# UM-Applied-Algorithms-Lab/AWRY

Hardware: AMD Instinct MI355X
Metric: k-mer count queries/sec (parallel_count, random 31-mers, index resident in HBM) (higher is better)
Workload: dtype u64

## Files before the change

### awry_amd/_lib.py

```python
import ctypes as C
import importlib.util
import os
import re

_HERE = os.path.dirname(os.path.abspath(__file__))
_SO = os.path.join(_HERE, "lib", "libawry_hip.so")
_HEADER = os.path.join(os.path.dirname(_HERE), "include", "awry_hip.h")
_lib = None


def lib_path():
    return _SO


class Pos(C.Structure):
    _fields_ = [("seq_idx", C.c_uint64), ("local_pos", C.c_uint64)]


class Range(C.Structure):
    _fields_ = [("start_ptr", C.c_uint64), ("end_ptr", C.c_uint64)]


class Anchor(C.Structure):
    _fields_ = [("q_begin", C.c_uint32), ("q_len", C.c_uint32), ("start_row", C.c_uint64), ("count", C.c_uint64)]
# ... 69 lines not shown
            "there is no CPU fallback for the search path." % _SO)
    _preload_hip_runtime()
    L = C.CDLL(_SO)
    vp, u64, u8, i32, cp = C.c_void_p, C.c_uint64, C.c_uint8, C.c_int, C.c_char_p
    u64p, u8p = C.POINTER(C.c_uint64), C.POINTER(C.c_uint8)
    vpp = C.POINTER(vp)

    def sig(name, res, *args):
        f = getattr(L, name)
        f.restype, f.argtypes = res, list(args)

    sig("awry_last_error", cp)
    sig("awry_build", i32, C.POINTER(BuildArgs), vpp)
    sig("awry_build_from_text", i32, vp, u64, i32, u64, u8, u64p, C.POINTER(cp), u64, vpp)
    sig("awry_build_from_text_on", i32, vp, u64, i32, u64, u8, u64p, C.POINTER(cp), u64, i32, vpp)
    sig("awry_load", i32, cp, vpp)
    sig("awry_save", i32, vp, cp)
    sig("awry_free", None, vp)
    sig("awry_set_devices", i32, vp, C.POINTER(i32), i32)
    sig("awry_set_seed_kmer_len", i32, vp, i32)
    sig("awry_seed_kmer_len", i32, vp)
    sig("awry_debug_set_count_kernel", i32, i32)
    sig("awry_debug_force_wide_rows", i32, i32)
    sig("awry_debug_set_max_blocks", i32, i32)
    sig("awry_debug_max_blocks", i32)
    sig("awry_debug_dense_sa", vp, vp, i32)
    sig("awry_debug_accelerators", i32, vp, i32, C.POINTER(DebugAccel))
    sig("awry_debug_seed_rung", vp, vp, i32, i32)
    sig("awry_debug_set_ctx_extra_cap", i32, i32)
    sig("awry_count_schedule", cp, vp, i32)
    sig("awry_num_devices", i32, vp)
    sig("awry_replica_device", i32, vp, i32)
    sig("awry_count_batch", i32, vp, vp, u64p, u64, u64p)
    sig("awry_count_packed_kmers", i32, vp, u64p, u64, i32, u64p)
    sig("awry_locate_batch", i32, vp, vp, u64p, u64, C.POINTER(u64p), C.POINTER(C.POINTER(Pos)), C.POINTER(u64p))
    sig("awry_free_buffer", None, vp)
    sig("awry_count_mismatch_batch", i32, vp, vp, u64p, u64, i32, u64p)
    sig("awry_locate_mismatch_batch", i32, vp, vp, u64p, u64, i32, C.POINTER(u64p), C.POINTER(C.POINTER(Pos)), C.POINTER(u64p),
        C.POINTER(u8p))
    sig("awry_dev_count_mismatch", i32, vp, i32, vp, vp, u64, i32, vp, vp, vp)
    sig("awry_dev_count_mismatch_tally", i32, vp, i32, vp, vp, u64, i32, vp, vp, vp, vp)
    u32 = C.c_uint32
    sig("awry_pattern_class", u32, i32, u8)
    sig("awry_count_pattern_batch", i32, vp, vp, u64p, u64, i32, u64p)
    sig("awry_locate_pattern_batch", i32, vp, vp, u64p, u64, i32, C.POINTER(u64p), C.POINTER(C.POINTER(Pos)), C.POINTER(u64p),
        C.POINTER(u8p))
# ... 111 lines not shown
```

### awry_amd/csrc/awry_hip.hip

```cpp
#include "dev_common.h"
#include "replica.h"
#include "accelerators.h"
#include "launchers.h"
#include "host_count.h"
#include "host_locate.h"
#include "batch_host.h"
#include "mismatch_host.h"
#include "anchor_host.h"
#include "chain_host.h"
#include "edit_host.h"
#include "chain_align_host.h"
#include "map_host.h"
#include "split_host.h"
#include "pair_host.h"
#include "prewarm.h"

namespace {

template <class T>
T* malloc_array(size_t n) {
  const size_t bytes = std::max<size_t>(1, n) * sizeof(T);
  void* p = nullptr;
  if (bytes >= (8u << 20)) {
    if (posix_memalign(&p, 2u << 20, bytes) != 0) p = nullptr;
// ... 201 lines not shown
        });
      for (auto& t : pool) t.join();
      for (auto& e : errs) if (e) std::rethrow_exception(e);
    }
    idx->reps = std::move(reps);
    for (auto& r : idx->reps) prewarm_host_paths(*r);
  });
}

int awry_set_seed_kmer_len(awry_index_t* idx, int k) {
  return guarded([&] {
    require(idx != nullptr, "null index");
    require(k >= -1 && k <= 17, "seed k-mer length must be in -1..17 (amino: ..7)");
    idx->seed_k_request = k;
    for (size_t s = 0; s < idx->reps.size(); s++) {
      Replica& r = replica(idx, (int)s);
      build_seed(idx, r, k < 0 ? default_seed_k(idx->host) : k);
      sync_seed_mode(idx, r);
    }
  });
}

int awry_debug_set_count_kernel(int mode) { g_count_kernel.store(mode); return AWRY_OK; }
int awry_debug_force_wide_rows(int on) { g_force_wide.store(on ? 1 : 0); return AWRY_OK; }
int awry_debug_set_max_blocks(int blocks) {
  if (blocks < 0) { g_last_error = "awry_debug_set_max_blocks: negative bound"; return AWRY_ERR_ARG; }
  g_max_blocks.store(blocks);
  return AWRY_OK;
}
int awry_debug_max_blocks(void) { return g_max_blocks.load(); }

const char* awry_count_schedule(const awry_index_t* idx, int L) {
  if (!idx || idx->reps.empty()) return "";
  const CountFacts f = count_facts(*idx->reps[0]);
  const uint64_t n = 1u << 20;
  return plan_name(L > 32 ? plan_reads(f, n, L, true, false) : plan_kmers(f, n, L, true, false));
}

int awry_seed_kmer_len(const awry_index_t* idx) { return idx && !idx->reps.empty() ? idx->reps[0]->seed_k : 0; }
int awry_num_devices(const awry_index_t* idx) { return idx ? (int)idx->reps.size() : 0; }
int awry_replica_device(const awry_index_t* idx, int slot) {
  return idx && slot >= 0 && slot < (int)idx->reps.size() ? idx->reps[slot]->device : -1;
}

int awry_count_batch(awry_index_t* idx, const uint8_t* qbytes, const uint64_t* qoff, uint64_t n, uint64_t* counts_out) {
  return guarded([&] {
// ... 1047 lines not shown
```

### awry_amd/csrc/kernels_nt2_kmer.hip.h

```cpp
#pragma once

namespace awry {

__device__ __forceinline__ void tally_flush(unsigned long long* __restrict__ tally, uint32_t t_probe, uint32_t t_step, uint32_t t_blk) {
  atomicAdd(&tally[0], (unsigned long long)t_probe);
  atomicAdd(&tally[1], (unsigned long long)t_step);
  atomicAdd(&tally[2], (unsigned long long)t_blk);
}

template <bool USE_SEED, bool TALLY>
__global__ __launch_bounds__(256) void count_nt2_quad_kernel(DevIndex ix, const uint64_t* __restrict__ queries, uint64_t n, int L,
                                                             uint64_t* __restrict__ counts, unsigned long long* __restrict__ tally) {
  const int l = threadIdx.x & 3;
  const uint64_t nquads = ((uint64_t)gridDim.x * blockDim.x) >> 2;
  uint64_t q = ((uint64_t)blockIdx.x * blockDim.x + threadIdx.x) >> 2;
  const uint64_t* __restrict__ blocks = ix.blocks;
  const SeedEntry* __restrict__ seed = ix.seed;
  const int k = USE_SEED ? ix.seed_k : 1;
  const uint32_t cA = (uint32_t)ix.prefix_sums[1], cC = (uint32_t)ix.prefix_sums[2], cG = (uint32_t)ix.prefix_sums[3],
                 cN = (uint32_t)ix.prefix_sums[4], cT = (uint32_t)ix.prefix_sums[5], cEnd = (uint32_t)ix.prefix_sums[6];

  bool have = q < n;
  uint64_t w = have ? queries[q] : 0;
  bool fresh = true;
// ... 143 lines not shown
  if (TALLY && l == 0) {
    tally_flush(tally, t_probe, t_step, t_blk);
    atomicAdd(&tally[5], (unsigned long long)t_deep);
    if (VERIFY) {
      atomicAdd(&tally[3], (unsigned long long)t_vsa);
      atomicAdd(&tally[4], (unsigned long long)t_vtxt);
    }
  }
}

constexpr int VMULTI = 4;
constexpr int LCX_LANE_ROWS = 4;
constexpr int LCX_TAIL_MAX = 16;

struct Nt2Survivors {
  uint64_t* w;
  uint64_t* range;
  uint32_t* q;
  uint32_t* count;
  uint64_t cap;
  uint32_t* lf_count = nullptr;
};

template <bool TALLY, bool VERIFY>
__device__ __forceinline__ unsigned probe_block(const DevIndex& ix, const uint64_t* __restrict__ queries, uint64_t n, int L,
                                                uint64_t* __restrict__ counts, const Nt2Survivors& sv,
                                                unsigned long long* __restrict__ tally) {
  __shared__ unsigned int s_count;
  constexpr int VQ = 192;
  __shared__ uint64_t s_vw[VERIFY ? 4 : 1][VQ];
  __shared__ uint32_t s_vsp[VERIFY ? 4 : 1][VQ];
  __shared__ uint32_t s_vq[VERIFY ? 4 : 1][VQ];
  __shared__ uint8_t s_vn[VERIFY ? 4 : 1][VQ];
  if (threadIdx.x == 0) s_count = 0;
  if (blockIdx.x == 0 && threadIdx.x == 0 && sv.lf_count) *sv.lf_count = 0;
  __syncthreads();
  const int lane = threadIdx.x & 63, wv_id = threadIdx.x >> 6;
  const SeedEntry* __restrict__ seed = ix.seed;
  const int k = ix.seed_k, i0 = L - k, kshift = 2 * (L - k);
  const uint64_t kmask = (1ull << (2 * k)) - 1;
  const uint64_t stride = (uint64_t)gridDim.x * blockDim.x;
  const uint64_t lane_lt = (1ull << lane) - 1;
  const uint64_t region = (uint64_t)blockIdx.x * sv.cap;
  const bool pos = VERIFY && ix.seed_pos;
  const int cx = (int)ix.ctx_extra, clen = SEED_CTX_LEN + cx;
  const bool verify = VERIFY && (i0 >= 3 || (pos && i0 >= 1));
  const bool lcx = VERIFY && ix.lcx_key != nullptr && i0 >= 1;
  int vcount = 0;
  uint32_t t_vsa = 0, t_vtxt = 0, t_lcx = 0;
  auto drain = [&](int base, int cnt) {
    uint64_t w[2];
    uint32_t q[2], sp[2], nc[2], vp[2];
    bool on[2];
#pragma unroll
    for (int h = 0; h < 2; h++) {
      const int s = base + lane + 64 * h;
      on[h] = lane + 64 * h < cnt;
      w[h] = on[h] ? s_vw[VERIFY ? wv_id : 0][s] : 0;
      q[h] = on[h] ? s_vq[VERIFY ? wv_id : 0][s] : 0;
      sp[h] = on[h] ? s_vsp[VERIFY ? wv_id : 0][s] : 0;
      nc[h] = on[h] ? s_vn[VERIFY ? wv_id : 0][s] : 0;
      vp[h] = sp[h];
      if (on[h] && !(nc[h] & 0x80u) && !(pos && nc[h] == 1u)) { vp[h] = ix.dense_sa[sp[h]]; if (TALLY) t_vsa++; }
    }
#pragma unroll
    for (int h = 0; h < 2; h++) {
      if (!on[h]) continue;
      uint64_t value = 0;
      if (nc[h] & 0x80u) {
        const uint64_t want = (w[h] & ((1ull << (2 * i0)) - 1)) << (64 - 2 * i0);
        const uint32_t rows = nc[h] & 0x7Fu;
        const uint64_t* __restrict__ kp = ix.lcx_key + sp[h];
        const uint64_t k0 = kp[0], k1 = kp[1], k2 = rows > 2u ? kp[2] : ~want, k3 = rows > 3u ? kp[3] : ~want;
        const int sh = 64 - 2 * i0;
        value = (((k0 ^ want) >> sh) == 0) + (((k1 ^ want) >> sh) == 0) + (((k2 ^ want) >> sh) == 0) + (((k3 ^ want) >> sh) == 0);
        if (TALLY) t_lcx++;
        counts[q[h]] = value;
        continue;
      }
      for (uint32_t c = 0; c < nc[h]; c++) {
        const uint32_t p = c ? ix.dense_sa[sp[h] + c] : vp[h];
        if (TALLY && c) t_vsa++;
        if (p >= (uint32_t)i0) {
          if (TALLY) t_vtxt++;
          value += verify_part(ix.text4, (uint64_t)p - (uint64_t)i0, i0, 0, 0, w[h]) ? 0ull : 1ull;
        }
      }
      counts[q[h]] = value;
    }
  };
  constexpr int NQ = 4;
  for (uint64_t wbase = (uint64_t)blockIdx.x * blockDim.x + (threadIdx.x & ~63u); wbase < n; wbase += NQ * stride) {
    uint64_t qv[NQ], wv[NQ];
    SeedEntry ev[NQ];
#pragma unroll
    for (int h = 0; h < NQ; h++) {
      qv[h] = wbase + lane + (uint64_t)h * stride;
      wv[h] = qv[h] < n ? queries[qv[h]] : 0;
    }
#pragma unroll
    for (int h = 0; h < NQ; h++) {
      ev[h] = SeedEntry{1u, 0u};
      if (qv[h] < n) ev[h] = seed_probe(seed + ((wv[h] >> kshift) & kmask));
    }
#pragma unroll
    for (int h = 0; h < NQ; h++) {
      const bool valid = qv[h] < n;
      const uint64_t q = qv[h], w = wv[h];
      const SeedEntry e = ev[h];
      const uint32_t cnt = seed_cnt(e);
      bool survivor = false, queued = false, lcx_q = false;
      uint64_t value = 0;
      if (valid) {
        if (cnt == SEED_CNT_SAT) survivor = true;
        else if (cnt == 0u) value = 0;
        else if (i0 == 0) value = cnt;
        else if (cnt == 1u && pos && seed_has_ctx(e) && i0 <= clen) {
          value = (w & ((1ull << (2 * i0)) - 1)) == (seed_full_ctx(e, cx) >> (2 * (clen - i0))) ? 1ull : 0ull;
        } else if (cnt == 1u && pos && seed_has_ctx(e)) {
          queued = ((w >> (2 * (i0 - clen))) & ((1ull << (2 * clen)) - 1)) == seed_full_ctx(e, cx);
        } else if (cnt == 1u) {
          const uint32_t nc = (uint32_t)(w >> (2 * (i0 - 1))) & 3u;
          survivor = seed_sym(e) == (int)(nc == 3u ? 5u : nc + 1u);
          if (verify && survivor) { queued = true; survivor = false; }
        } else if (lcx && !(e.cnt & (SEED_LCX_NONE | SEED_LCX_TAIL)) && cnt <= (uint32_t)LCX_LANE_ROWS) {
          queued = true;
          lcx_q = true;
        } else if (lcx && !(e.cnt & SEED_LCX_NONE)) {
          survivor = true;
        } else if (verify && cnt <= (uint32_t)VMULTI && (int)(3u * cnt) <= i0 + 2) {
          queued = true;
        } else survivor = true;
        if (!queued) counts[q] = value;
      }
      if (VERIFY) {
        const uint64_t qm = __ballot(queued);
        if (qm) {
          if (queued) {
            const int s = vcount + (int)__popcll(qm & lane_lt);
            s_vw[wv_id][s] = w;
            s_vsp[wv_id][s] = cnt == 1u && pos ? seed_position(e, cx) : e.sp;
            s_vq[wv_id][s] = (uint32_t)q;
            s_vn[wv_id][s] = (uint8_t)(cnt | (lcx_q ? 0x80u : 0u));
          }
          vcount += (int)__popcll(qm);
          __builtin_amdgcn_wave_barrier();
          if (vcount >= 128) {
            vcount -= 128;
            drain(vcount, 128);
            __builtin_amdgcn_wave_barrier();
          }
        }
      }
      const uint64_t sm = __ballot(survivor);
      if (sm) {
        unsigned int slot0 = 0;
        if (lane == 0) slot0 = atomicAdd(&s_count, (unsigned int)__popcll(sm));
        slot0 = __shfl(slot0, 0, 64);
        if (survivor) {
          const uint64_t s = region + slot0 + (uint64_t)__popcll(sm & lane_lt);
          sv.w[s] = w;
          sv.range[s] = (uint64_t)e.sp | ((uint64_t)(cnt | (e.cnt & (SEED_LCX_NONE | SEED_LCX_TAIL))) << 32);
          sv.q[s] = (uint32_t)q;
        }
      }
    }
  }
  if (VERIFY && vcount > 0) drain(0, vcount);
  if (TALLY) {
    if (blockIdx.x == 0 && threadIdx.x == 0) atomicAdd(&tally[0], (unsigned long long)n);
    if (VERIFY && (t_vsa | t_vtxt | t_lcx)) {
      atomicAdd(&tally[3], (unsigned long long)t_vsa);
      atomicAdd(&tally[4], (unsigned long long)t_vtxt);
      atomicAdd(&tally[6], (unsigned long long)t_lcx);
    }
  }
  __syncthreads();
  return s_count;
}

template <bool TALLY, bool VERIFY>
__global__ __launch_bounds__(256) void count_nt2_probe_kernel(DevIndex ix, const uint64_t* __restrict__ queries, uint64_t n, int L,
                                                              uint64_t* __restrict__ counts, Nt2Survivors sv,
                                                              unsigned long long* __restrict__ tally) {
  const unsigned ns = probe_block<TALLY, VERIFY>(ix, queries, n, L, counts, sv, tally);
  if (threadIdx.x == 0) sv.count[blockIdx.x] = ns;
}

template <bool TALLY, bool VERIFY, bool TABLE = false>
__device__ __forceinline__ void resume_block_list(const DevIndex& ix, const Nt2Survivors& sv, uint64_t region, uint64_t ns, int L,
                                                  uint64_t* __restrict__ counts, unsigned long long* __restrict__ tally, bool allow_lcx,
                                                  uint64_t r_start, uint64_t r_stride) {
  const int l = threadIdx.x & 3;
  uint64_t r = r_start;
  const uint64_t* __restrict__ blocks = ix.blocks;
  const int k = ix.seed_k;
  const int verify_after = (int)ix.verify_after;
// ... 20 lines not shown
        if (fresh) {
          w = nx_w;
          const uint64_t rg = nx_rg;
          qidx = nx_q;
          if (r + r_stride < ns) { nx_w = sv.w[region + r + r_stride]; nx_rg = sv.range[region + r + r_stride]; nx_q = sv.q[region + r + r_stride]; }
          const uint32_t cf = (uint32_t)(rg >> 32), cnt = cf & SEED_CNT_SAT;
          steps_done = 0;
          fresh = false;
          if (qidx == 0xFFFFFFFFu) {
            sp = 1u; ep = 0u; i = 0;
          } else if (cnt == SEED_CNT_SAT) {
            const uint32_t c = (uint32_t)(w >> (2 * (L - 1))) & 3u;
            sp = c == 0 ? cA : (c == 1 ? cC : (c == 2 ? cG : cT));
            ep = (c == 0 ? cC : (c == 1 ? cG : (c == 2 ? cN : cEnd))) - 1;
            i = L - 1;
          } else {
            sp = (uint32_t)rg;
            ep = sp + cnt - 1u;
            i = L - k;
            if (lcx && cnt >= 2u && !(cf & SEED_LCX_NONE) && i > 0) {
              steps_done = 0;
              if (cf & SEED_LCX_TAIL) mode = 3;
              else { vp = ub_a = sp; vhits = ub_b = sp + cnt; vj = lcx_top_level(sp, cnt); mode = 4; }
              if (TABLE && ix.kmer_tab && cnt > (uint32_t)LCX_LANE_ROWS) { steps_done = mode; mode = 7; }
            }
          }
        }
        if (mode == 0) {
          const bool skip_step = VERIFY && i > 0 && sp <= ep && verify_now(ep - sp + 1u, i, steps_done, verify_after);
          if (i > 0 && sp <= ep && !skip_step) {
            i--;
            const uint32_t c = (uint32_t)(w >> (2 * i)) & 3u;
            const uint32_t cl = c == 0 ? cA : (c == 1 ? cC : (c == 2 ? cG : cT));
            if (TALLY) { t_step++; t_blk += ((sp - 1) >> 8) == (ep >> 8) ? 1u : 2u; }
            quad_step(blocks, cl, sp, ep, c, l);
            steps_done++;
          }
          if (sp > ep || i == 0) {
            finished = true;
            out_count = sp > ep ? 0ull : (uint64_t)(ep - sp) + 1ull;
          } else if (VERIFY) {
            const uint32_t cnt = ep - sp + 1u;
            if (verify_now(cnt, i, steps_done, verify_after)) { mode = 1; vj = 0; vhits = 0; }
          }
        }
      } else if (mode == 1) {
        vp = ix.dense_sa[sp + (uint32_t)vj];
// ... 68 lines not shown
    }
  }
  if (TALLY && l == 0) {
    atomicAdd(&tally[1], (unsigned long long)t_step);
    atomicAdd(&tally[2], (unsigned long long)t_blk);
    if (VERIFY) {
      atomicAdd(&tally[3], (unsigned long long)t_vsa);
      atomicAdd(&tally[4], (unsigned long long)t_vtxt);
      atomicAdd(&tally[6], (unsigned long long)t_lcx);
      atomicAdd(&tally[7], (unsigned long long)t_rp);
    }
  }
}

template <bool TALLY, bool VERIFY>
__global__ __launch_bounds__(256) void count_nt2_resume_kernel(DevIndex ix, Nt2Survivors sv, int L, uint64_t* __restrict__ counts,
                                                               unsigned long long* __restrict__ tally) {
  resume_block_list<TALLY, VERIFY>(ix, sv, (uint64_t)blockIdx.x * sv.cap, (uint64_t)sv.count[blockIdx.x], L, counts, tally, true, threadIdx.x >> 2, 64);
}

template <bool TALLY, bool VERIFY>
__global__ __launch_bounds__(256) void count_nt2_probe_resume_kernel(DevIndex ix, const uint64_t* __restrict__ queries, uint64_t n, int L, uint64_t* __restrict__ counts,
                                   Nt2Survivors sv, unsigned long long* __restrict__ tally) {
  const unsigned ns = probe_block<TALLY, VERIFY>(ix, queries, n, L, counts, sv, tally);
  resume_block_list<TALLY, VERIFY, true>(ix, sv, (uint64_t)blockIdx.x * sv.cap, (uint64_t)ns, L, counts, tally, true, threadIdx.x >> 2, 64);
}
constexpr int NT2_CHUNK = 256;

template <bool USE_SEED, bool TALLY>
__global__ __launch_bounds__(256) void count_nt2_chunk_kernel(DevIndex ix, const uint64_t* __restrict__ queries, uint64_t n, int L,
                                                              uint64_t* __restrict__ counts, unsigned long long* __restrict__ chunk_counter,
                                                              unsigned long long* __restrict__ tally) {
  __shared__ uint64_t lds_all[4 * NT2_CHUNK];
  const int lane = threadIdx.x & 63, l = lane & 3;
  volatile uint64_t* lds = lds_all + (threadIdx.x >> 6) * NT2_CHUNK;
  const uint64_t* __restrict__ blocks = ix.blocks;
  const SeedEntry* __restrict__ seed = ix.seed;
  const int k = USE_SEED ? ix.seed_k : 1;
  const uint32_t cA = (uint32_t)ix.prefix_sums[1], cC = (uint32_t)ix.prefix_sums[2], cG = (uint32_t)ix.prefix_sums[3],
                 cN = (uint32_t)ix.prefix_sums[4], cT = (uint32_t)ix.prefix_sums[5], cEnd = (uint32_t)ix.prefix_sums[6];
  const uint64_t nchunks = (n + NT2_CHUNK - 1) / NT2_CHUNK;
  const uint64_t quad_lt = (1ull << (lane & ~3)) - 1;
  uint32_t t_probe = 0, t_step = 0, t_blk = 0;

  for (;;) {
    unsigned long long c = 0;
    if (lane == 0) c = atomicAdd(chunk_counter, 1ull);
// ... 69 lines not shown
```

### awry_amd/csrc/kmer_table.hip.h

```cpp
#pragma once

namespace awry {

__device__ __forceinline__ void kt_add(uint64_t* __restrict__ table, uint32_t bits, uint64_t key, int L, uint64_t n, unsigned long long* __restrict__ stats) {
  const uint64_t mx = kt_mix(key, L);
  unsigned long long* line = reinterpret_cast<unsigned long long*>(table) + ((mx & ((1ull << bits) - 1)) << 4);
  const uint64_t tag = mx >> bits;
  for (int u = tag >= KT_TAG_NONE ? 16 : 0; u < 16;) {
    const unsigned long long e = __hip_atomic_load(line + u, __ATOMIC_RELAXED, __HIP_MEMORY_SCOPE_AGENT);
    const uint64_t cnt = e & KT_CNT_MASK;
    if (cnt == 0) {
      const uint64_t c = n < KT_ASK ? n : KT_ASK;
      if (atomicCAS(line + u, e, (tag << KT_TAG_SHIFT) | (e & KT_OVERFLOW) | c) == e) { atomicAdd(&stats[0], 1ull); return; }
      continue;
    }
    if ((e >> KT_TAG_SHIFT) == tag) {
      const uint64_t c = cnt + n < KT_ASK ? cnt + n : KT_ASK;
      if (atomicCAS(line + u, e, (e & ~KT_CNT_MASK) | c) == e) return;
      continue;
    }
    u++;
  }
  if (!(atomicOr(line, (unsigned long long)KT_OVERFLOW) & KT_OVERFLOW)) atomicAdd(&stats[1], 1ull);
}

template <bool INSERT>
__global__ __launch_bounds__(256) void kt_scan_kernel(DevIndex ix, int L, uint64_t* __restrict__ table, uint32_t bits, unsigned long long* __restrict__ stats) {
  const int k = ix.seed_k, i0 = L - k, sh = 64 - 2 * i0;
  const uint64_t stride = (uint64_t)gridDim.x * blockDim.x;
  unsigned long long mine = 0;
  for (uint64_t r = (uint64_t)blockIdx.x * blockDim.x + threadIdx.x; r < ix.bwt_len; r += stride) {
    const uint32_t p = ix.dense_sa[r];
    bool ok = false;
    const uint64_t kmer = lcx_text_letters(ix.text4, p, k, &ok);
    if (!ok) continue;
    const SeedEntry e = ix.seed[kmer];
    if (seed_has_ctx(e) || (e.cnt & SEED_LCX_NONE)) continue;
    const uint32_t cnt = e.cnt & SEED_CNT_SAT;
    if (cnt <= (uint32_t)LCX_LANE_ROWS || cnt == SEED_CNT_SAT) continue;
    const uint32_t sp = e.sp, j = (uint32_t)r - sp;
    if (r < sp || j >= cnt) continue;
    const uint32_t inc = (e.cnt & SEED_LCX_TAIL) ? (uint32_t)ix.lcx_key[sp + cnt - 1u] : 0u;
    const uint32_t nc = cnt - (inc < cnt ? inc : cnt);
    if (j < nc) {
// ... 31 lines not shown
```

### awry_amd/csrc/launchers.h

```cpp
#pragma once

namespace {

std::atomic<int> g_count_kernel{-1};
int count_kernel_override() {
  int m = g_count_kernel.load();
  if (m >= 0) return m;
  const char* e = getenv("AWRY_COUNT_KERNEL");
  if (e && !strcmp(e, "strided")) return 0;
  if (e && !strcmp(e, "chunk")) return 1;
  if (e && !strcmp(e, "quad4")) return 2;
  if (e && !strcmp(e, "twophase")) return 3;
  return -1;
}

CountFacts count_facts(const Replica& r) {
  static const bool rungs_off = getenv("AWRY_SEED_RUNGS") && !strcmp(getenv("AWRY_SEED_RUNGS"), "0");
  static const bool table_off = getenv("AWRY_KMER_TABLE") && !strcmp(getenv("AWRY_KMER_TABLE"), "0");
  CountFacts f;
  f.alphabet = r.dev.alphabet;
  f.wide = r.wide;
  f.bwt_len = r.dev.bwt_len;
  f.seed_k = r.seed_k;
  f.seed = r.seed.p != nullptr;
  f.seed64 = r.dev.seed64 != nullptr;
  f.text4 = r.dev.text4 != nullptr;
  f.dense_ratio = r.dev.dense_ratio;
  f.lcx_key = r.dev.lcx_key != nullptr;
  f.kt_mode = r.kt_mode;
  f.verify_kmers = r.verify_kmers;
  f.num_cus = r.num_cus;
  for (int i = 0; i < 4; i++) f.probe_resume_per_cu[i] = r.probe_resume_per_cu[i];
  for (int i = 0; i < 2; i++) f.lcx_reads_grid[i] = r.lcx_reads_grid[i];
  f.forced = count_kernel_override();
  f.rungs_off = rungs_off;
  f.table_off = table_off;
// ... 182 lines not shown
      });
      break;
    }
    default: require(false, "internal: not a schedule for reads");
  }
  HIP_CHECK(hipGetLastError());
}

void launch_count_nt2(Replica& r, const uint64_t* d_words, uint64_t n, int L, uint64_t* d_counts, bool use_seed, hipStream_t s,
                      unsigned long long* d_tally = nullptr) {
  require(r.dev.alphabet == NUCLEOTIDE, "packed 2-bit queries need a nucleotide index");
  require(L >= 1 && L <= 32, "packed k-mer length must be in 1..32");
  if (n == 0) return;
  const ScratchLock scratch_lock(r, s);
  CountFacts f = count_facts(r);
  CountPlan p = plan_kmers(f, n, L, use_seed, d_tally != nullptr);
  DevIndex dv = r.dev;
  std::shared_lock<std::shared_mutex> kt_lock;
  if (p.rung) {
    if (const SeedEntry* t = seed_rung(r, L)) { dv.seed = t; dv.seed_k = L; dv.seed_pos = 0; dv.ctx_extra = 0; }
    else { f.rung_failed = true; p = plan_kmers(f, n, L, use_seed, d_tally != nullptr); }
  }
  if (p.table) {
    if (const Replica::KmerTable* kt = kmer_table(r, L, true, kt_lock)) { dv.kmer_tab = kt->tab.p; dv.kmer_tab_bits = kt->bits; }
    else { f.table_failed = true; p = plan_kmers(f, n, L, use_seed, d_tally != nullptr); }
  }
  const dim3 g(plan_grid(r, p, n)), b(256);
  switch (p.schedule) {
    case CountSchedule::WIDE_SINGLE:
    case CountSchedule::WIDE_TWO_PHASE:
      launch_count_nt2_wide(r, p, d_words, n, L, d_counts, nullptr, s, nullptr, d_tally);
      return;
    case CountSchedule::LDS_CHUNKS: {
      unsigned long long* ctr = next_counter(r, s);
      with_flags(p.seeded, d_tally != nullptr, [&](auto S, auto T) {
        hipLaunchKernelGGL((count_nt2_chunk_kernel<S(), T()>), g, b, 0, s, r.dev, d_words, n, L, d_counts, ctr, d_tally);
      });
      break;
    }
    case CountSchedule::PROBE_RESUME:
    case CountSchedule::PROBE_THEN_RESUME: {
      Nt2Survivors sv, fb;
      two_phase_lists(r, s, n, p.blocks, 0u, &sv, &fb);
      with_flags(d_tally != nullptr, p.verify, [&](auto T, auto V) {
        if (p.schedule == CountSchedule::PROBE_THEN_RESUME) {
          hipLaunchKernelGGL((count_nt2_probe_kernel<T(), V()>), g, b, 0, s, dv, d_words, n, L, d_counts, sv, d_tally);
          hipLaunchKernelGGL((count_nt2_resume_kernel<T(), V()>), g, b, 0, s, dv, sv, L, d_counts, d_tally);
// ... 339 lines not shown
```

### awry_amd/csrc/layout.h

```cpp
#pragma once
#include <stdint.h>

#if defined(__HIP__)
#define AWRY_HD __host__ __device__ inline __attribute__((always_inline))
#else
#define AWRY_HD inline
#endif

namespace awry {

enum : int { NUCLEOTIDE = 0, AMINO = 1 };

constexpr int NT_BLOCK_WORDS = 16;
constexpr int AA_BLOCK_WORDS = 32;
constexpr int SYMBOLS_PER_BLOCK = 256;

AWRY_HD int block_words(int alphabet) { return alphabet == NUCLEOTIDE ? NT_BLOCK_WORDS : AA_BLOCK_WORDS; }
AWRY_HD int num_planes(int alphabet) { return alphabet == NUCLEOTIDE ? 3 : 5; }
AWRY_HD int cardinality(int alphabet) { return alphabet == NUCLEOTIDE ? 6 : 22; }

AWRY_HD int plane_word(int alphabet, int b, int l) {
  if (alphabet == NUCLEOTIDE) return b < 2 ? 2 * l + b : 8 + 2 * l;
  return b < 2 ? 2 * l + b : (b < 4 ? 8 + 2 * l + (b - 2) : 16 + 2 * l);
}
// ... 48 lines not shown
  const uint64_t* sa_words;
  const SeedEntry* seed;
  const SeedEntry64* seed64;
  const uint64_t* seq_starts;
  const uint32_t* seq_bucket;
  uint32_t seq_bucket_shift, seq_bucket_pad;
  uint64_t nblocks, bwt_len, sentinel_row, nseq;
  uint64_t prefix_sums[24];
  uint32_t sa_bits, sa_ratio;
  int32_t alphabet, seed_k;
  const uint32_t* dense_sa;
  const uint32_t* text4;
  uint32_t dense_ratio;
  uint32_t verify_after;
  const uint8_t* text8;
  uint32_t ctx_extra;
  uint32_t seed_pos;
  const uint32_t* sa_nblock;
  const uint64_t* lcx_key;
  const uint64_t* lcx_rowpos;
  const uint64_t* lcx_inner;
  uint32_t lcx_off[8];
  const uint64_t* kmer_tab;
  uint32_t kmer_tab_bits, kmer_tab_pad;
};
constexpr int LCX_CTX = 32;

constexpr int KT_CNT_BITS = 20, KT_TAG_SHIFT = 21, KT_TAG_BITS = 64 - KT_TAG_SHIFT;
constexpr uint64_t KT_CNT_MASK = (1ull << KT_CNT_BITS) - 1, KT_ASK = KT_CNT_MASK, KT_OVERFLOW = 1ull << KT_CNT_BITS;
constexpr uint64_t KT_TAG_NONE = (1ull << KT_TAG_BITS) - 1;
AWRY_HD uint64_t kt_mix(uint64_t w, int L) {
  const uint64_t m = L >= 32 ? ~0ull : (1ull << (2 * L)) - 1;
  w = (w * 0x9E3779B97F4A7C15ull) & m;
  w ^= w >> L;
  w = (w * 0xD6E8FEB86659FD93ull) & m;
  w ^= w >> L;
  return w;
}

constexpr uint64_t RS_MODE_SHIFT = 62;
constexpr uint64_t RS_PLAIN = 0;
constexpr uint64_t RS_MULTI = 1;
constexpr uint64_t RS_SINGLE = 2;
constexpr uint64_t RS_LCX = 3;

constexpr int LIST_MAX_LISTS = 4096;
constexpr int LCX_LF_CHUNK = 256;

}
```

### awry_amd/fm_index.py

```python
import ctypes as C
import os
from dataclasses import dataclass
from typing import Iterable, List, Optional, Sequence

import numpy as np

from . import _lib

NUCLEOTIDE, AMINO = 0, 1
BUILD_HOST, BUILD_AUTO = -1, -2


class SymbolAlphabet:
    Nucleotide = NUCLEOTIDE
    Amino = AMINO


class AwryError(RuntimeError):
    def __init__(self, code, msg):
        super().__init__("awry error %d: %s" % (code, msg))
        self.code = code


ERR_IO, ERR_FORMAT, ERR_INVALID_QUERY, ERR_HIP, ERR_OOM, ERR_ARG, ERR_NO_DEVICE = -1, -2, -3, -4, -5, -6, -7
# ... 939 lines not shown
    def dev_locate_tally(self, d_ranges, d_hit_off, n, total, d_gpos, d_pos, d_tally, stream=None, slot=0, range_stride=2):
        _check(self._L.awry_dev_locate_tally(self._h, slot, d_ranges, range_stride, d_hit_off, n, total, d_gpos, d_pos, d_tally, stream))

    def dev_phase_marker(self, phase_id, stream=None, slot=0):
        _check(self._L.awry_dev_phase_marker(self._h, slot, phase_id, stream))

    def dev_count_nt2_long(self, d_words, n, L, d_counts, d_range_start=None, use_seed=True, stream=None, slot=0):
        _check(self._L.awry_dev_count_nt2_long(self._h, slot, d_words, n, L, d_counts, d_range_start, 1 if use_seed else 0, stream))

    def set_locate_sa_ratio(self, ratio: int):
        _check(self._L.awry_set_locate_sa_ratio(self._h, ratio))

    def locate_sa_ratio(self) -> int:
        return self._L.awry_locate_sa_ratio(self._h)

    def set_lcx(self, on: bool):
        _check(self._L.awry_set_lcx(self._h, 1 if on else 0))

    def lcx_enabled(self) -> bool:
        return bool(self._L.awry_lcx_enabled(self._h))

    def set_kmer_table(self, mode: int):
        _check(self._L.awry_set_kmer_table(self._h, mode))

    def kmer_table_info(self, slot=0) -> dict:
        info = (C.c_uint64 * 6)()
        _check(self._L.awry_kmer_table_info(self._h, slot, info))
        return {"length": int(info[0]), "entries": int(info[1]), "lines": int(info[2]), "overflowed_lines": int(info[3]),
                "bytes": int(info[4]), "build_ms": int(info[5]) / 1000.0}

    def debug_kmer_table(self, slot=0):
        L, bits = C.c_int(0), C.c_uint32(0)
        for _ in range(4):
            _check(self._L.awry_debug_kmer_table(self._h, slot, None, 0, C.byref(L), C.byref(bits)))
            if L.value == 0:
                return None
            want = bits.value
            tab = np.empty(16 << want, np.uint64)
            _check(self._L.awry_debug_kmer_table(self._h, slot, tab.ctypes.data, len(tab), C.byref(L), C.byref(bits)))
            if L.value == 0:
                return None
            if bits.value <= want:
                return tab[:16 << bits.value], int(bits.value), int(L.value)
        raise AwryError(ERR_ARG, "the k-mer count table kept changing size while it was read")

    def debug_lcx(self, slot=0):
# ... 114 lines not shown
```

### include/awry_hip.h

```cpp
#ifndef AWRY_HIP_H
#define AWRY_HIP_H
#include <stddef.h>
#include <stdint.h>

#ifdef __cplusplus
extern "C" {
#endif

enum {
  AWRY_OK = 0,
  AWRY_ERR_IO = -1,
  AWRY_ERR_FORMAT = -2,
  AWRY_ERR_INVALID_QUERY = -3,
  AWRY_ERR_HIP = -4,
  AWRY_ERR_OOM = -5,
  AWRY_ERR_ARG = -6,
  AWRY_ERR_NO_DEVICE = -7
};

enum { AWRY_NUCLEOTIDE = 0, AWRY_AMINO = 1 };

typedef struct awry_index awry_index_t;

typedef struct { uint64_t seq_idx, local_pos; } awry_pos_t;
// ... 6 lines not shown
  uint64_t sa_ratio;
  uint8_t kmer_len;
  uint8_t alphabet;
  uint64_t max_query_len;
  uint8_t remove_tmp;
} awry_build_args_t;

int awry_build(const awry_build_args_t *args, awry_index_t **out);
int awry_build_from_text(const uint8_t *text, uint64_t bwt_len, int alphabet, uint64_t sa_ratio, uint8_t kmer_len,
                         const uint64_t *seq_starts, const char *const *headers, uint64_t nseq, awry_index_t **out);
enum { AWRY_BUILD_HOST = -1, AWRY_BUILD_AUTO = -2 };
int awry_build_from_text_on(const uint8_t *text, uint64_t bwt_len, int alphabet, uint64_t sa_ratio, uint8_t kmer_len,
                            const uint64_t *seq_starts, const char *const *headers, uint64_t nseq, int build_device,
                            awry_index_t **out);
int awry_load(const char *path, awry_index_t **out);
int awry_save(awry_index_t *idx, const char *path);
void awry_free(awry_index_t *idx);

int awry_set_devices(awry_index_t *idx, const int *device_ids, int n_devices);
int awry_set_seed_kmer_len(awry_index_t *idx, int k);
int awry_seed_kmer_len(const awry_index_t *idx);
int awry_debug_set_count_kernel(int mode);
int awry_debug_force_wide_rows(int on);
int awry_debug_set_max_blocks(int blocks);
int awry_debug_max_blocks(void);
const void *awry_debug_dense_sa(const awry_index_t *idx, int slot);
typedef struct {
  const void *seed;
  int32_t seed_k, seed_entry_bytes, seed_pos, ctx_extra;
  const void *dense_sa;
  uint64_t dense_ratio;
  const void *text4;
  uint64_t text4_words;
  const void *text8;
  const void *sa_nblock;
  uint64_t nblock_lo, nblock_hi;
  const void *lcx_inner;
  uint64_t lcx_inner_words;
  uint32_t lcx_off[8];
} awry_debug_accel_t;
int awry_debug_accelerators(const awry_index_t *idx, int slot, awry_debug_accel_t *out);
const void *awry_debug_seed_rung(awry_index_t *idx, int slot, int L);
int awry_debug_set_ctx_extra_cap(int cap);
const char *awry_count_schedule(const awry_index_t *idx, int L);
int awry_set_locate_sa_ratio(awry_index_t *idx, int ratio);
int awry_locate_sa_ratio(const awry_index_t *idx);
// ... 298 lines not shown
```

### rust/awry-hip-sys/src/lib.rs

```rust
#![allow(non_camel_case_types)]
use std::os::raw::{c_char, c_int, c_void};

pub const AWRY_OK: c_int = 0;
pub const AWRY_ERR_IO: c_int = -1;
pub const AWRY_ERR_FORMAT: c_int = -2;
pub const AWRY_ERR_INVALID_QUERY: c_int = -3;
pub const AWRY_ERR_HIP: c_int = -4;
pub const AWRY_ERR_OOM: c_int = -5;
pub const AWRY_ERR_ARG: c_int = -6;
pub const AWRY_ERR_NO_DEVICE: c_int = -7;
pub const AWRY_NUCLEOTIDE: c_int = 0;
pub const AWRY_AMINO: c_int = 1;
pub const AWRY_BUILD_HOST: c_int = -1;
pub const AWRY_BUILD_AUTO: c_int = -2;

#[repr(C)]
pub struct awry_index_t {
    _private: [u8; 0],
}

#[repr(C)]
#[derive(Clone, Copy, Debug, Default, PartialEq, Eq)]
pub struct awry_pos_t {
    pub seq_idx: u64,
// ... 146 lines not shown
pub struct awry_build_args_t {
    pub input_path: *const c_char,
    pub sa_tmp_path: *const c_char,
    pub sa_ratio: u64,
    pub kmer_len: u8,
    pub alphabet: u8,
    pub max_query_len: u64,
    pub remove_tmp: u8,
}

#[link(name = "awry_hip")]
extern "C" {
    pub fn awry_build(args: *const awry_build_args_t, out: *mut *mut awry_index_t) -> c_int;
    pub fn awry_build_from_text(text: *const u8, bwt_len: u64, alphabet: c_int, sa_ratio: u64, kmer_len: u8, seq_starts: *const u64, headers: *const *const c_char, nseq: u64, out: *mut *mut awry_index_t) -> c_int;
    pub fn awry_build_from_text_on(text: *const u8, bwt_len: u64, alphabet: c_int, sa_ratio: u64, kmer_len: u8, seq_starts: *const u64, headers: *const *const c_char, nseq: u64, build_device: c_int, out: *mut *mut awry_index_t) -> c_int;
    pub fn awry_load(path: *const c_char, out: *mut *mut awry_index_t) -> c_int;
    pub fn awry_save(idx: *mut awry_index_t, path: *const c_char) -> c_int;
    pub fn awry_free(idx: *mut awry_index_t);
    pub fn awry_set_devices(idx: *mut awry_index_t, device_ids: *const c_int, n_devices: c_int) -> c_int;
    pub fn awry_set_seed_kmer_len(idx: *mut awry_index_t, k: c_int) -> c_int;
    pub fn awry_seed_kmer_len(idx: *const awry_index_t) -> c_int;
    pub fn awry_debug_set_count_kernel(mode: c_int) -> c_int;
    pub fn awry_debug_force_wide_rows(on: c_int) -> c_int;
    pub fn awry_debug_set_max_blocks(blocks: c_int) -> c_int;
    pub fn awry_debug_max_blocks() -> c_int;
    pub fn awry_debug_dense_sa(idx: *const awry_index_t, slot: c_int) -> *const c_void;
    pub fn awry_debug_accelerators(idx: *const awry_index_t, slot: c_int, out: *mut awry_debug_accel_t) -> c_int;
    pub fn awry_debug_seed_rung(idx: *mut awry_index_t, slot: c_int, L: c_int) -> *const c_void;
    pub fn awry_debug_set_ctx_extra_cap(cap: c_int) -> c_int;
    pub fn awry_count_schedule(idx: *const awry_index_t, L: c_int) -> *const c_char;
    pub fn awry_set_locate_sa_ratio(idx: *mut awry_index_t, ratio: c_int) -> c_int;
    pub fn awry_locate_sa_ratio(idx: *const awry_index_t) -> c_int;
    pub fn awry_set_verify(idx: *mut awry_index_t, after_steps: c_int) -> c_int;
    pub fn awry_set_verify_kmers(idx: *mut awry_index_t, on: c_int) -> c_int;
    pub fn awry_verify_enabled(idx: *const awry_index_t) -> c_int;
    pub fn awry_set_lcx(idx: *mut awry_index_t, on: c_int) -> c_int;
    pub fn awry_lcx_enabled(idx: *const awry_index_t) -> c_int;
    pub fn awry_debug_lcx(idx: *const awry_index_t, slot: c_int, d_keys: *mut *const c_void, d_rowpos: *mut *const c_void) -> c_int;
    pub fn awry_set_kmer_table(idx: *mut awry_index_t, mode: c_int) -> c_int;
    pub fn awry_kmer_table_info(idx: *mut awry_index_t, slot: c_int, info: *mut u64) -> c_int;
    pub fn awry_debug_set_kmer_table_lines(lines: u64) -> c_int;
    pub fn awry_debug_kmer_table(idx: *mut awry_index_t, slot: c_int, host_out: *mut u64, capacity_words: u64, L_out: *mut c_int, bits_out: *mut u32) -> c_int;
    pub fn awry_num_devices(idx: *const awry_index_t) -> c_int;
    pub fn awry_count_batch(idx: *mut awry_index_t, qbytes: *const u8, qoff: *const u64, n: u64, counts_out: *mut u64) -> c_int;
    pub fn awry_count_packed_kmers(idx: *mut awry_index_t, words: *const u64, n: u64, L: c_int, counts_out: *mut u64) -> c_int;
    pub fn awry_locate_batch(idx: *mut awry_index_t, qbytes: *const u8, qoff: *const u64, n: u64, hit_off_out: *mut *mut u64, hits_out: *mut *mut awry_pos_t, global_pos_out: *mut *mut u64) -> c_int;
// ... 99 lines not shown
```

Before: 39.21 billion.

## Resolve k-mer hash-table lookups per lane in probe phase before survivor resume

Adds a per-lane k-mer count table lookup inside the probe block's drain step. Queries whose seed range exceeds the lane-row limit are queued for a direct table probe instead of being written out as survivors for the later resume phase. Only table misses, ask-markers and overflow cases fall back to the survivor list, tagged so resume does not look them up again. The table probe start slot is now spread by tag bits in both insert and lookup, to lower clustering within a 16-slot line. The change cuts survivor traffic and resume work, at the cost of extra register and shared-memory pressure and more divergent loops in the probe kernel.

```diff
diff --git a/awry_amd/_lib.py b/awry_amd/_lib.py
--- a/awry_amd/_lib.py
+++ b/awry_amd/_lib.py
@@ -115,6 +115,7 @@
     sig("awry_seed_kmer_len", i32, vp)
     sig("awry_debug_set_count_kernel", i32, i32)
     sig("awry_debug_force_wide_rows", i32, i32)
+    sig("awry_debug_set_kmer_lane_lookup", i32, i32)
     sig("awry_debug_set_max_blocks", i32, i32)
     sig("awry_debug_max_blocks", i32)
     sig("awry_debug_dense_sa", vp, vp, i32)
diff --git a/awry_amd/csrc/awry_hip.hip b/awry_amd/csrc/awry_hip.hip
--- a/awry_amd/csrc/awry_hip.hip
+++ b/awry_amd/csrc/awry_hip.hip
@@ -247,6 +247,7 @@
 }
 
 int awry_debug_set_count_kernel(int mode) { g_count_kernel.store(mode); return AWRY_OK; }
+int awry_debug_set_kmer_lane_lookup(int on) { g_kmer_lane.store(on < 0 ? -1 : (on ? 1 : 0)); return AWRY_OK; }
 int awry_debug_force_wide_rows(int on) { g_force_wide.store(on ? 1 : 0); return AWRY_OK; }
 int awry_debug_set_max_blocks(int blocks) {
   if (blocks < 0) { g_last_error = "awry_debug_set_max_blocks: negative bound"; return AWRY_ERR_ARG; }
diff --git a/awry_amd/csrc/kernels_nt2_kmer.hip.h b/awry_amd/csrc/kernels_nt2_kmer.hip.h
--- a/awry_amd/csrc/kernels_nt2_kmer.hip.h
+++ b/awry_amd/csrc/kernels_nt2_kmer.hip.h
@@ -189,7 +189,10 @@
   uint32_t* lf_count = nullptr;
 };
 
-template <bool TALLY, bool VERIFY>
+constexpr int KT_LANE_INFLIGHT = 2;
+constexpr uint32_t KT_QUEUED = 0x40u;
+constexpr uint32_t SV_TABLE_ASKED = 0x80000000u;
+template <bool TALLY, bool VERIFY, bool TABLE = false>
 __device__ __forceinline__ unsigned probe_block(const DevIndex& ix, const uint64_t* __restrict__ queries, uint64_t n, int L,
                                                 uint64_t* __restrict__ counts, const Nt2Survivors& sv,
                                                 unsigned long long* __restrict__ tally) {
@@ -213,8 +216,9 @@
   const int cx = (int)ix.ctx_extra, clen = SEED_CTX_LEN + cx;
   const bool verify = VERIFY && (i0 >= 3 || (pos && i0 >= 1));
   const bool lcx = VERIFY && ix.lcx_key != nullptr && i0 >= 1;
+  const bool kt_lane = TABLE && lcx && ix.kmer_tab != nullptr && ix.kmer_tab_lane != 0;
   int vcount = 0;
-  uint32_t t_vsa = 0, t_vtxt = 0, t_lcx = 0;
+  uint32_t t_vsa = 0, t_vtxt = 0, t_lcx = 0, t_kt = 0;
   auto drain = [&](int base, int cnt) {
     uint64_t w[2];
     uint32_t q[2], sp[2], nc[2], vp[2];
@@ -228,11 +232,11 @@
       sp[h] = on[h] ? s_vsp[VERIFY ? wv_id : 0][s] : 0;
       nc[h] = on[h] ? s_vn[VERIFY ? wv_id : 0][s] : 0;
       vp[h] = sp[h];
-      if (on[h] && !(nc[h] & 0x80u) && !(pos && nc[h] == 1u)) { vp[h] = ix.dense_sa[sp[h]]; if (TALLY) t_vsa++; }
+      if (on[h] && !(nc[h] & (0x80u | KT_QUEUED)) && !(pos && nc[h] == 1u)) { vp[h] = ix.dense_sa[sp[h]]; if (TALLY) t_vsa++; }
     }
 #pragma unroll
     for (int h = 0; h < 2; h++) {
-      if (!on[h]) continue;
+      if (!on[h] || (TABLE && (nc[h] & KT_QUEUED))) continue;
       uint64_t value = 0;
       if (nc[h] & 0x80u) {
         const uint64_t want = (w[h] & ((1ull << (2 * i0)) - 1)) << (64 - 2 * i0);
@@ -255,6 +259,69 @@
       }
       counts[q[h]] = value;
     }
+    if (TABLE && kt_lane && __any((nc[0] | nc[1]) & KT_QUEUED)) {
+      __asm__ volatile("" ::: "memory");
+      uint64_t kw[2];
+      uint32_t mark[2];
+      ulonglong2 x[2], y[2];
+      bool kt[2], back[2];
+      const uint64_t lmask = (1ull << ix.kmer_tab_bits) - 1;
+#pragma unroll
+      for (int g = 0; g < 2; g += KT_LANE_INFLIGHT) {
+#pragma unroll
+      for (int h = g; h < g + KT_LANE_INFLIGHT; h++) {
+        const int s = base + lane + 64 * h;
+        kt[h] = lane + 64 * h < cnt && (s_vn[VERIFY ? wv_id : 0][s] & KT_QUEUED);
+        if (!kt[h]) continue;
+        kw[h] = s_vw[VERIFY ? wv_id : 0][s];
+        const uint64_t mx = kt_mix(kw[h], L);
+        const uint64_t* line = ix.kmer_tab + ((mx & lmask) << 4);
+        const ulonglong2* sec = reinterpret_cast<const ulonglong2*>(line + kt_probe_slot(mx >> ix.kmer_tab_bits, 0));
+        mark[h] = *reinterpret_cast<const uint32_t*>(line);
+        x[h] = sec[0];
+        y[h] = sec[1];
+        if (TALLY) t_lcx++;
+      }
+#pragma unroll
+      for (int h = g; h < g + KT_LANE_INFLIGHT; h++) {
+        back[h] = false;
+        if (!kt[h]) continue;
+        const uint64_t mx = kt_mix(kw[h], L), tag = mx >> ix.kmer_tab_bits;
+        const uint64_t want = tag >= KT_TAG_NONE ? ~0ull : tag << KT_TAG_SHIFT;
+        uint32_t found = 0;
+        for (int j = 0;;) {
+          found = (((x[h].x ^ want) >> KT_TAG_SHIFT) == 0 ? (uint32_t)x[h].x & (uint32_t)KT_CNT_MASK : 0u) +
+                  (((x[h].y ^ want) >> KT_TAG_SHIFT) == 0 ? (uint32_t)x[h].y & (uint32_t)KT_CNT_MASK : 0u) +
+                  (((y[h].x ^ want) >> KT_TAG_SHIFT) == 0 ? (uint32_t)y[h].x & (uint32_t)KT_CNT_MASK : 0u) +
+                  (((y[h].y ^ want) >> KT_TAG_SHIFT) == 0 ? (uint32_t)y[h].y & (uint32_t)KT_CNT_MASK : 0u);
+          const bool empty = !((uint32_t)x[h].x & (uint32_t)KT_CNT_MASK) || !((uint32_t)x[h].y & (uint32_t)KT_CNT_MASK) ||
+                             !((uint32_t)y[h].x & (uint32_t)KT_CNT_MASK) || !((uint32_t)y[h].y & (uint32_t)KT_CNT_MASK);
+          j += 4;
+          if (found || empty || j == 16) break;
+          const ulonglong2* sec = reinterpret_cast<const ulonglong2*>(ix.kmer_tab + ((mx & lmask) << 4) + kt_probe_slot(tag, j));
+          x[h] = sec[0];
+          y[h] = sec[1];
+        }
+        back[h] = found == (uint32_t)KT_ASK || (found == 0u && (mark[h] & (uint32_t)KT_OVERFLOW));
+        if (!back[h]) { counts[s_vq[VERIFY ? wv_id : 0][base + lane + 64 * h]] = found; if (TALLY) t_kt++; }
+      }
+      }
+#pragma unroll
+      for (int h = 0; h < 2; h++) {
+        const uint64_t bm = __ballot(back[h]);
+        if (!bm) continue;
+        unsigned int slot0 = 0;
+        if (lane == 0) slot0 = atomicAdd(&s_count, (unsigned int)__popcll(bm));
+        slot0 = __shfl(slot0, 0, 64);
+        if (back[h]) {
+          const SeedEntry e = seed_probe(seed + ((kw[h] >> kshift) & kmask));
+          const uint64_t s = region + slot0 + (uint64_t)__popcll(bm & lane_lt);
+          sv.w[s] = kw[h];
+          sv.range[s] = (uint64_t)e.sp | ((uint64_t)((e.cnt & (SEED_CNT_SAT | SEED_LCX_NONE | SEED_LCX_TAIL)) | SV_TABLE_ASKED) << 32);
+          sv.q[s] = s_vq[VERIFY ? wv_id : 0][base + lane + 64 * h];
+        }
+      }
+    }
   };
   constexpr int NQ = 4;
   for (uint64_t wbase = (uint64_t)blockIdx.x * blockDim.x + (threadIdx.x & ~63u); wbase < n; wbase += NQ * stride) {
@@ -276,7 +343,7 @@
       const uint64_t q = qv[h], w = wv[h];
       const SeedEntry e = ev[h];
       const uint32_t cnt = seed_cnt(e);
-      bool survivor = false, queued = false, lcx_q = false;
+      bool survivor = false, queued = false, lcx_q = false, kt_q = false;
       uint64_t value = 0;
       if (valid) {
         if (cnt == SEED_CNT_SAT) survivor = true;
@@ -294,7 +361,8 @@
           queued = true;
           lcx_q = true;
         } else if (lcx && !(e.cnt & SEED_LCX_NONE)) {
-          survivor = true;
+          if (TABLE && kt_lane && cnt > (uint32_t)LCX_LANE_ROWS) queued = kt_q = true;
+          else survivor = true;
         } else if (verify && cnt <= (uint32_t)VMULTI && (int)(3u * cnt) <= i0 + 2) {
           queued = true;
         } else survivor = true;
@@ -308,7 +376,7 @@
             s_vw[wv_id][s] = w;
             s_vsp[wv_id][s] = cnt == 1u && pos ? seed_position(e, cx) : e.sp;
             s_vq[wv_id][s] = (uint32_t)q;
-            s_vn[wv_id][s] = (uint8_t)(cnt | (lcx_q ? 0x80u : 0u));
+            s_vn[wv_id][s] = TABLE && kt_q ? (uint8_t)KT_QUEUED : (uint8_t)(cnt | (lcx_q ? 0x80u : 0u));
           }
           vcount += (int)__popcll(qm);
           __builtin_amdgcn_wave_barrier();
@@ -340,6 +408,7 @@
       atomicAdd(&tally[3], (unsigned long long)t_vsa);
       atomicAdd(&tally[4], (unsigned long long)t_vtxt);
       atomicAdd(&tally[6], (unsigned long long)t_lcx);
+      if (TABLE && t_kt) atomicAdd(&tally[5], (unsigned long long)t_kt);
     }
   }
   __syncthreads();
@@ -406,7 +475,7 @@
               steps_done = 0;
               if (cf & SEED_LCX_TAIL) mode = 3;
               else { vp = ub_a = sp; vhits = ub_b = sp + cnt; vj = lcx_top_level(sp, cnt); mode = 4; }
-              if (TABLE && ix.kmer_tab && cnt > (uint32_t)LCX_LANE_ROWS) { steps_done = mode; mode = 7; }
+              if (TABLE && ix.kmer_tab && cnt > (uint32_t)LCX_LANE_ROWS && !(cf & SV_TABLE_ASKED)) { steps_done = mode; mode = 7; }
             }
           }
         }
@@ -521,7 +590,7 @@
 template <bool TALLY, bool VERIFY>
 __global__ __launch_bounds__(256) void count_nt2_probe_resume_kernel(DevIndex ix, const uint64_t* __restrict__ queries, uint64_t n, int L, uint64_t* __restrict__ counts,
                                    Nt2Survivors sv, unsigned long long* __restrict__ tally) {
-  const unsigned ns = probe_block<TALLY, VERIFY>(ix, queries, n, L, counts, sv, tally);
+  const unsigned ns = probe_block<TALLY, VERIFY, true>(ix, queries, n, L, counts, sv, tally);
   resume_block_list<TALLY, VERIFY, true>(ix, sv, (uint64_t)blockIdx.x * sv.cap, (uint64_t)ns, L, counts, tally, true, threadIdx.x >> 2, 64);
 }
 constexpr int NT2_CHUNK = 256;
diff --git a/awry_amd/csrc/kmer_table.hip.h b/awry_amd/csrc/kmer_table.hip.h
--- a/awry_amd/csrc/kmer_table.hip.h
+++ b/awry_amd/csrc/kmer_table.hip.h
@@ -6,7 +6,8 @@
   const uint64_t mx = kt_mix(key, L);
   unsigned long long* line = reinterpret_cast<unsigned long long*>(table) + ((mx & ((1ull << bits) - 1)) << 4);
   const uint64_t tag = mx >> bits;
-  for (int u = tag >= KT_TAG_NONE ? 16 : 0; u < 16;) {
+  for (int j = tag >= KT_TAG_NONE ? 16 : 0; j < 16;) {
+    const int u = kt_probe_slot(tag, j);
     const unsigned long long e = __hip_atomic_load(line + u, __ATOMIC_RELAXED, __HIP_MEMORY_SCOPE_AGENT);
     const uint64_t cnt = e & KT_CNT_MASK;
     if (cnt == 0) {
@@ -19,7 +20,7 @@
       if (atomicCAS(line + u, e, (e & ~KT_CNT_MASK) | c) == e) return;
       continue;
     }
-    u++;
+    j++;
   }
   if (!(atomicOr(line, (unsigned long long)KT_OVERFLOW) & KT_OVERFLOW)) atomicAdd(&stats[1], 1ull);
 }
diff --git a/awry_amd/csrc/launchers.h b/awry_amd/csrc/launchers.h
--- a/awry_amd/csrc/launchers.h
+++ b/awry_amd/csrc/launchers.h
@@ -12,6 +12,14 @@
   if (e && !strcmp(e, "quad4")) return 2;
   if (e && !strcmp(e, "twophase")) return 3;
   return -1;
+}
+
+std::atomic<int> g_kmer_lane{-1};
+bool kmer_lane_lookup() {
+  const int m = g_kmer_lane.load();
+  if (m >= 0) return m != 0;
+  static const bool off = getenv("AWRY_KMER_LANE") && !strcmp(getenv("AWRY_KMER_LANE"), "0");
+  return !off;
 }
 
 CountFacts count_facts(const Replica& r) {
@@ -240,7 +248,7 @@
     else { f.rung_failed = true; p = plan_kmers(f, n, L, use_seed, d_tally != nullptr); }
   }
   if (p.table) {
-    if (const Replica::KmerTable* kt = kmer_table(r, L, true, kt_lock)) { dv.kmer_tab = kt->tab.p; dv.kmer_tab_bits = kt->bits; }
+    if (const Replica::KmerTable* kt = kmer_table(r, L, true, kt_lock)) { dv.kmer_tab = kt->tab.p; dv.kmer_tab_bits = kt->bits; dv.kmer_tab_lane = kmer_lane_lookup() ? 1u : 0u; }
     else { f.table_failed = true; p = plan_kmers(f, n, L, use_seed, d_tally != nullptr); }
   }
   const dim3 g(plan_grid(r, p, n)), b(256);
diff --git a/awry_amd/csrc/layout.h b/awry_amd/csrc/layout.h
--- a/awry_amd/csrc/layout.h
+++ b/awry_amd/csrc/layout.h
@@ -94,7 +94,8 @@
   const uint64_t* lcx_inner;
   uint32_t lcx_off[8];
   const uint64_t* kmer_tab;
-  uint32_t kmer_tab_bits, kmer_tab_pad;
+  uint32_t kmer_tab_bits;
+  uint32_t kmer_tab_lane;
 };
 constexpr int LCX_CTX = 32;
 
@@ -109,6 +110,7 @@
   w ^= w >> L;
   return w;
 }
+AWRY_HD int kt_probe_slot(uint64_t tag, int j) { return (int)((((uint32_t)tag & 3u) * 4u + (uint32_t)j) & 15u); }
 
 constexpr uint64_t RS_MODE_SHIFT = 62;
 constexpr uint64_t RS_PLAIN = 0;
diff --git a/awry_amd/fm_index.py b/awry_amd/fm_index.py
--- a/awry_amd/fm_index.py
+++ b/awry_amd/fm_index.py
@@ -985,6 +985,10 @@
 
     def set_kmer_table(self, mode: int):
         _check(self._L.awry_set_kmer_table(self._h, mode))
+
+    @staticmethod
+    def debug_set_kmer_lane_lookup(on: int):
+        _check(_lib.load_library().awry_debug_set_kmer_lane_lookup(int(on)))
 
     def kmer_table_info(self, slot=0) -> dict:
         info = (C.c_uint64 * 6)()
diff --git a/include/awry_hip.h b/include/awry_hip.h
--- a/include/awry_hip.h
+++ b/include/awry_hip.h
@@ -52,6 +52,7 @@
 int awry_seed_kmer_len(const awry_index_t *idx);
 int awry_debug_set_count_kernel(int mode);
 int awry_debug_force_wide_rows(int on);
+int awry_debug_set_kmer_lane_lookup(int on);
 int awry_debug_set_max_blocks(int blocks);
 int awry_debug_max_blocks(void);
 const void *awry_debug_dense_sa(const awry_index_t *idx, int slot);
diff --git a/rust/awry-hip-sys/src/lib.rs b/rust/awry-hip-sys/src/lib.rs
--- a/rust/awry-hip-sys/src/lib.rs
+++ b/rust/awry-hip-sys/src/lib.rs
@@ -192,6 +192,7 @@
     pub fn awry_seed_kmer_len(idx: *const awry_index_t) -> c_int;
     pub fn awry_debug_set_count_kernel(mode: c_int) -> c_int;
     pub fn awry_debug_force_wide_rows(on: c_int) -> c_int;
+    pub fn awry_debug_set_kmer_lane_lookup(on: c_int) -> c_int;
     pub fn awry_debug_set_max_blocks(blocks: c_int) -> c_int;
     pub fn awry_debug_max_blocks() -> c_int;
     pub fn awry_debug_dense_sa(idx: *const awry_index_t, slot: c_int) -> *const c_void;
```

After: 39.75 billion, median of 5. 1.01x the previous value.
